# jirsat/wavenets

Measured on NVIDIA B200. Metric: audio samples/sec fwd+bwd WaveNet stack, higher is better.
Workload: dtype bf16

## Files before the change

wavenets_b200/csrc/gemm_tc_block.cuh:

```cuda
#pragma once
#include "gemm_tc.cuh"

template <int NT1> __device__ __forceinline__ void blk_tile(int pos, int n, int& kind, int& j) {
  if (pos < NT1) { kind = pos; j = 0; return; }
  const int q = (pos - NT1) / (NT1 + 1), r = (pos - NT1) % (NT1 + 1);
  if (q >= n - 1) { kind = NT1; j = n - 1; return; }
  if (r == 0) { kind = 0; j = q + 1; }
  else if (r == 1) { kind = NT1; j = q; }
  else { kind = r - 1; j = q + 1; }
}

struct TcBlockParams {
  int B, T, tiles_t, num_mtiles;
  int nseg, shift[TC_MAX_TAPS];
  int Cin, D, R, has_res;
  const float* bias_g; const float* cbias; const float* bias_r;
  unsigned long long pol_a, pol_w, pol_z, pol_g, pol_o;
  float drop_scale;
};

template <int D_, int R_> struct TcBlockCfg {
  static constexpr int BM = 128, BK = 64, BN = 256;
  static constexpr int A_BYTES = BM * BK * 2;
  static constexpr int B_BYTES = (BN / 2) * BK * 2;
  static constexpr int STAGE_BYTES = A_BYTES + B_BYTES;
  static constexpr int STAGES = 4;
  static constexpr int G_BYTES = BM * D_ * 2;
  static constexpr int PANEL = 128 * 64;
  static constexpr int OUT_SLOTS = 2, SLOT_PANELS = 2;
  static constexpr int NT1 = 2 * D_ / BN;
  static constexpr int TMEM_COLS = 512;
  static constexpr int SMEM_BYTES = STAGES * STAGE_BYTES + G_BYTES + OUT_SLOTS * SLOT_PANELS * PANEL + 512  + 2048 ;
  static_assert(D_ % 128 == 0 && D_ <= 256 && R_ % 64 == 0 && R_ <= 256, "fused block kernel: D in {128,256}, R <= 256");
  static_assert(SMEM_BYTES <= 232448, "fused block kernel does not fit shared memory");
};

template <int D_, int R_>
__global__ void __launch_bounds__(384, 1)
tc_block_fwd_kernel(const __grid_constant__ CUtensorMap tmA, const __grid_constant__ CUtensorMap tmX, const __grid_constant__ CUtensorMap tmW1,
                    const __grid_constant__ CUtensorMap tmW2, const __grid_constant__ CUtensorMap tmZf, const __grid_constant__ CUtensorMap tmZs,
                    const __grid_constant__ CUtensorMap tmG, const __grid_constant__ CUtensorMap tmO, const TcBlockParams p) {
  using Cfg = TcBlockCfg<D_, R_>;
  constexpr int STAGES = Cfg::STAGES, NEPI = 8, NT1 = Cfg::NT1;
  constexpr int KB_G = D_ / 64, KB_X = R_ / 64;
  extern __shared__ __align__(1024) uint8_t smem_blk[];
  uint8_t* smem = smem_blk;
  if ((smem_u32(smem) & 1023u) != 0u) { if (threadIdx.x == 0) printf("libwavenet_b200: dynamic shared memory is not 1024-byte aligned\n"); __trap(); }
  uint8_t* gbuf = smem + STAGES * Cfg::STAGE_BYTES;
  uint8_t* out_ring = gbuf + Cfg::G_BYTES;
  uint64_t* full_bar = (uint64_t*)(out_ring + Cfg::OUT_SLOTS * Cfg::SLOT_PANELS * Cfg::PANEL);
  uint64_t* empty_bar = full_bar + STAGES;
  uint64_t* tfull_bar = empty_bar + STAGES;
  uint64_t* tempty_bar = tfull_bar + 2;
  uint64_t* out_empty = tempty_bar + 2;
  uint64_t* g_done = out_empty + Cfg::OUT_SLOTS;
  uint64_t* g_full = g_done + 1;
  uint64_t* g_free = g_full + 1;
  uint64_t* g_cons = g_free + 1;
  uint32_t* tmem_ptr = (uint32_t*)(g_cons + 2);
  float* bias_s = (float*)(((uintptr_t)(tmem_ptr + 4) + 15) & ~(uintptr_t)15);

  const int warp = threadIdx.x >> 5, lane = threadIdx.x & 31;
  const uint32_t crank = cluster_ctarank();
  const bool leader = crank == 0;
  const int tile_first = (int)blockIdx.x >> 1, tile_stride = (int)gridDim.x >> 1;
  const int pair_row0 = (int)crank * Cfg::BM;
  const int kb_a = p.Cin / 64;
  const int n_mt = tile_first < p.num_mtiles ? (p.num_mtiles - tile_first + tile_stride - 1) / tile_stride : 0;
  const int n_pos = n_mt * (NT1 + 1);

  if (warp == 0 && lane == 0) {
    tma_prefetch_desc(&tmA); tma_prefetch_desc(&tmW1); tma_prefetch_desc(&tmW2); tma_prefetch_desc(&tmX);
  }
  if (warp == 1 && lane == 0) {
    for (int i = 0; i < STAGES; ++i) { mbar_init(&full_bar[i], 1); mbar_init(&empty_bar[i], 1); }
    for (int i = 0; i < 2; ++i) { mbar_init(&tfull_bar[i], 1); mbar_init(&tempty_bar[i], NEPI * 2); }
    for (int i = 0; i < Cfg::OUT_SLOTS; ++i) mbar_init(&out_empty[i], 1);
    mbar_init(g_done, NEPI); mbar_init(g_full, 2); mbar_init(g_free, 1); mbar_init(&g_cons[0], 1); mbar_init(&g_cons[1], 1);
    mbar_fence_init();
  }
  if (warp == 2) tmem_alloc_pair<Cfg::TMEM_COLS>(tmem_ptr);
  tc_fence_before();
  __syncthreads();
  cluster_sync_all();
  tc_fence_after();
  const uint32_t tmem_base = *tmem_ptr;
  pdl_launch_dependents();
  pdl_wait();

  if (warp == 0) {
    if (lane == 0) {
      int stage = 0; uint32_t phase = 0;
      auto next = [&]() { if (++stage == STAGES) { stage = 0; phase ^= 1; } };
      constexpr int W2_BYTES = (R_ / 2) * 64 * 2;
      for (int pos = 0; pos < n_pos; ++pos) {
// ... 2 lines not shown
        const int mt = tile_first + j * tile_stride;
        const int b = mt / p.tiles_t, t0 = (mt % p.tiles_t) * (2 * Cfg::BM) + pair_row0;
        if (kind < NT1) {
          int wk = 0;
          for (int s = 0; s < p.nseg; ++s) {
            for (int kb = 0; kb < kb_a; ++kb) {
              mbar_wait(&empty_bar[stage], phase ^ 1);
              uint8_t* sa = smem + stage * Cfg::STAGE_BYTES;
              if (leader) mbar_expect_tx(&full_bar[stage], 2 * Cfg::STAGE_BYTES);
              tma_load_4d_pair_h(sa, &tmA, &full_bar[stage], kb * 64, t0 + p.shift[s], b, 0, p.pol_a);
              tma_load_2d_pair_h(sa + Cfg::A_BYTES, &tmW1, &full_bar[stage], wk + kb * 64, kind * Cfg::BN + (int)crank * (Cfg::BN / 2), p.pol_w);
              next();
            }
            wk += p.Cin;
          }
        } else {
          for (int kb = 0; kb < KB_G; ++kb) {
            mbar_wait(&empty_bar[stage], phase ^ 1);
            uint8_t* sa = smem + stage * Cfg::STAGE_BYTES;
            if (leader) mbar_expect_tx(&full_bar[stage], 2 * W2_BYTES);
            tma_load_2d_pair_h(sa + Cfg::A_BYTES, &tmW2, &full_bar[stage], kb * 64, (int)crank * (R_ / 2), p.pol_w);
            next();
          }
          if (p.has_res) {
            for (int kb = 0; kb < KB_X; ++kb) {
              mbar_wait(&empty_bar[stage], phase ^ 1);
              uint8_t* sa = smem + stage * Cfg::STAGE_BYTES;
              if (leader) mbar_expect_tx(&full_bar[stage], 2 * (Cfg::A_BYTES + W2_BYTES));
              tma_load_4d_pair_h(sa, &tmX, &full_bar[stage], kb * 64, t0, b, 0, p.pol_a);
              tma_load_2d_pair_h(sa + Cfg::A_BYTES, &tmW2, &full_bar[stage], D_ + kb * 64, (int)crank * (R_ / 2), p.pol_w);
              next();
            }
          }
        }
      }
    }
  } else if (warp == 1) {
    if (leader) {
      constexpr uint32_t idesc_g = umma_idesc_bf16(256, Cfg::BN, 0, 0);
      constexpr uint32_t idesc_o = umma_idesc_bf16(256, R_, 0, 0);
      int stage = 0; uint32_t phase = 0;
      int as = 0; uint32_t aphase = 0;
      uint32_t gphase = 0;
      const int ksteps_g = p.nseg * kb_a;
      const int ksteps_o = KB_G + (p.has_res ? KB_X : 0);
#ifdef TC_TIMELINE
      long long tl_rec[12][4]; int tl_n = 0; const long long tl_start = clock64();
#endif
      for (int pos = 0; pos < n_pos; ++pos) {
        {
          int kind, j;
          blk_tile<NT1>(pos, n_mt, kind, j);
          const bool is_out = kind == NT1;
          const int ksteps = is_out ? ksteps_o : ksteps_g;
#ifdef TC_TIMELINE
          const long long tl0 = clock64();
#endif
          mbar_wait(&tempty_bar[as], aphase ^ 1);
#ifdef TC_TIMELINE
          const long long tl1 = clock64();
#endif
          if (is_out) { mbar_wait(g_full, gphase); gphase ^= 1; }
#ifdef TC_TIMELINE
          const long long tl2 = clock64();
#endif
          tc_fence_after();
          const uint32_t d_tmem = tmem_base + (uint32_t)(as * Cfg::BN);
          for (int ks = 0; ks < ksteps; ++ks) {
            mbar_wait(&full_bar[stage], phase);
            tc_fence_after();
            if (elect_one()) {
              const uint32_t sa = smem_u32(smem + stage * Cfg::STAGE_BYTES);
              const uint32_t a_addr = (is_out && ks < KB_G) ? smem_u32(gbuf) + (uint32_t)ks * (uint32_t)Cfg::A_BYTES : sa;
              const uint64_t adesc = umma_smem_desc(a_addr, 16, 1024);
              const uint64_t bdesc = umma_smem_desc(sa + Cfg::A_BYTES, 16, 1024);
#pragma unroll
              for (int k = 0; k < Cfg::BK / 16; ++k)
                umma_bf16_pair(d_tmem, adesc + (uint64_t)(2 * k), bdesc + (uint64_t)(2 * k), is_out ? idesc_o : idesc_g, (ks | k) != 0);
              umma_commit_pair(&empty_bar[stage]);
              if (ks == ksteps - 1) umma_commit_pair(&tfull_bar[as]);
              if (is_out && ks < KB_G && (ks + 1) % (KB_G / NT1) == 0) umma_commit_pair(&g_cons[(ks + 1) / (KB_G / NT1) - 1]);
            }
            __syncwarp();
            if (++stage == STAGES) { stage = 0; phase ^= 1; }
          }
#ifdef TC_TIMELINE
          if (tl_n < 12) { tl_rec[tl_n][0] = tl1 - tl0; tl_rec[tl_n][1] = tl2 - tl1; tl_rec[tl_n][2] = clock64() - tl2; tl_rec[tl_n][3] = tl0 - tl_start; ++tl_n; }
#endif
          if (++as == 2) { as = 0; aphase ^= 1; }
        }
      }
#ifdef TC_TIMELINE
      if (blockIdx.x == 0 && lane == 0)
        for (int i = 0; i < tl_n; ++i) printf("BLK mma tile %d: t0 %lld wait_tempty %lld wait_g %lld issue %lld\n", i, tl_rec[i][3], tl_rec[i][0], tl_rec[i][1], tl_rec[i][2]);
#endif
    }
  } else if (warp == 2) {
    int oslot = 0, prev = -1;
    auto step_store = [&](const CUtensorMap* m0, const CUtensorMap* m1, int c0, int t0, int b, unsigned long long pol) {
      named_bar_sync(3 + oslot, NEPI * 32 + 32);
      if (lane == 0) {
        const uint8_t* ob = out_ring + oslot * Cfg::SLOT_PANELS * Cfg::PANEL;
        tma_store_3d_h(ob, m0, c0, t0, b, pol);
        if (m1) tma_store_3d_h(ob + Cfg::PANEL, m1, c0, t0, b, pol);
// ... 47 lines not shown
    const uint32_t u0 = (uint32_t)(2 * q), u1 = u0 + 1;
    const uint32_t off0 = row_off + ((u0 ^ sw) << 4), off1 = row_off + ((u1 ^ sw) << 4);
    const uint32_t grow = (uint32_t)row * 128u, gsw = (uint32_t)(row & 7);
    int as = 0; uint32_t aphase = 0;
    int oslot = 0; uint32_t ophase = 0;

#ifdef TC_TIMELINE
    long long tl_rec[12][3]; int tl_n = 0; const long long tl_start = clock64();
#endif
    const TcEpiGate<true>::Params pg{p.bias_g, p.cbias, D_};
    const TcEpiBiasActRes<true>::Params po{p.bias_r, nullptr, 0, ACT_LINEAR, R_};
    for (int pos = 0; pos < n_pos; ++pos) {
      int nt, j;
      blk_tile<NT1>(pos, n_mt, nt, j);
      const int mt = tile_first + j * tile_stride;
      const int b = mt / p.tiles_t;
      const int bsafe = b < p.B ? b : p.B - 1;
      {
        const bool is_out = nt == NT1;
        const int tid = (int)threadIdx.x - 128;
        float bias_reg = 0.f;
        if (is_out) { if (tid < R_) bias_reg = TcEpiBiasActRes<true>::bias_load(po, bsafe, 0, R_, tid); }
        else bias_reg = TcEpiGate<true>::bias_load(pg, bsafe, nt * (Cfg::BN / 2), Cfg::BN, tid);
#ifdef TC_TIMELINE
        const long long te0 = clock64();
#endif
        mbar_wait(&tfull_bar[as], aphase);
        tc_fence_after();
#ifdef TC_TIMELINE
        const long long te1 = clock64();
#endif
        float* const bs = bias_s + as * 256;
        bs[tid] = bias_reg;
        named_bar_sync(2, NEPI * 32);
        TmemAccRow acc{tmem_base + (uint32_t)(as * Cfg::BN) + ((uint32_t)(quarter * 32) << 16), true};
        if (!is_out) {
          if (j > 0) {
            mbar_wait(&g_cons[nt], (uint32_t)((j - 1) & 1));
            if (nt == 0) mbar_wait(g_free, (uint32_t)((j - 1) & 1));
          }
#pragma unroll 1
          for (int step = 0; step < Cfg::BN / 64; ++step) {
            float in[1][16];
            float out[3][16];
            TcEpiGate<true>::chunk(pg, acc, bsafe, step * 32 + q * 16, Cfg::BN / 2, 0, 0u, in, out, bs);
            uint8_t* ob = out_ring + oslot * Cfg::SLOT_PANELS * Cfg::PANEL;
// ... 12 lines not shown
              const int ch = nt * (Cfg::BN / 2) + step * 32 + q * 16;
              uint8_t* gs = gbuf + (ch >> 6) * Cfg::A_BYTES + grow;
              const uint32_t j0 = (uint32_t)((ch & 63) >> 3);
              uint4 a, c;
              a.x = pack_bf16x2(out[2][0], out[2][1]); a.y = pack_bf16x2(out[2][2], out[2][3]);
              a.z = pack_bf16x2(out[2][4], out[2][5]); a.w = pack_bf16x2(out[2][6], out[2][7]);
              c.x = pack_bf16x2(out[2][8], out[2][9]); c.y = pack_bf16x2(out[2][10], out[2][11]);
              c.z = pack_bf16x2(out[2][12], out[2][13]); c.w = pack_bf16x2(out[2][14], out[2][15]);
              *reinterpret_cast<uint4*>(gs + ((j0 ^ gsw) << 4)) = a;
              *reinterpret_cast<uint4*>(gs + (((j0 + 1) ^ gsw) << 4)) = c;
            }
            fence_proxy_async();
            named_bar_arrive(3 + oslot, NEPI * 32 + 32);
            if (++oslot == Cfg::OUT_SLOTS) { oslot = 0; ophase ^= 1; }
          }
          if (nt == NT1 - 1) {
            named_bar_arrive(8, NEPI * 32 + 32);
            __syncwarp();
            if (lane == 0) mbar_arrive(g_done);
          }
        } else {
#pragma unroll 1
          for (int step = 0; step < R_ / 32; ++step) {
            float in[1][16];
            float out[1][16];
            TcEpiBiasActRes<true>::chunk(po, acc, bsafe, step * 32 + q * 16, 0, 0, 0u, in, out, bs);
            uint8_t* ob = out_ring + oslot * Cfg::SLOT_PANELS * Cfg::PANEL;
            mbar_wait(&out_empty[oslot], ophase ^ 1);
            uint4 a, c;
            a.x = pack_bf16x2(out[0][0], out[0][1]); a.y = pack_bf16x2(out[0][2], out[0][3]);
            a.z = pack_bf16x2(out[0][4], out[0][5]); a.w = pack_bf16x2(out[0][6], out[0][7]);
            c.x = pack_bf16x2(out[0][8], out[0][9]); c.y = pack_bf16x2(out[0][10], out[0][11]);
            c.z = pack_bf16x2(out[0][12], out[0][13]); c.w = pack_bf16x2(out[0][14], out[0][15]);
            *reinterpret_cast<uint4*>(ob + off0) = a;
            *reinterpret_cast<uint4*>(ob + off1) = c;
            fence_proxy_async();
            named_bar_arrive(3 + oslot, NEPI * 32 + 32);
            if (++oslot == Cfg::OUT_SLOTS) { oslot = 0; ophase ^= 1; }
          }
        }
#ifdef TC_TIMELINE
        if (tl_n < 12) { tl_rec[tl_n][0] = te1 - te0; tl_rec[tl_n][1] = clock64() - te1; tl_rec[tl_n][2] = te0 - tl_start; ++tl_n; }
#endif
        tc_fence_before();
        __syncwarp();
        if (lane == 0) mbar_arrive_remote_relaxed(&tempty_bar[as], 0u);
        if (++as == 2) { as = 0; aphase ^= 1; }
      }
    }
// ... 11 lines not shown
struct TcBlockDesc {
  int B, T, nseg, shift[TC_MAX_TAPS], Cin, D, R, has_res;
  const bf16* A; int lda;
  const bf16* X; int ldx;
  const bf16* W1; int k1;
  const bf16* W2;
  bf16* z; bf16* g; bf16* xout;
  const float* bias_g; const float* cbias; const float* bias_r;
  const uint8_t* mask_next; bf16* xdrop_next; float drop_scale;
  int plain, act;
};

static inline const CUtensorMap* tc_slab_map(TmapCache& tc, const bf16* base, int ld, int C, int T, int B) {
  uint64_t dims[3] = {(uint64_t)C, (uint64_t)T, (uint64_t)B};
  uint64_t str[2] = {(uint64_t)ld * 2, (uint64_t)T * ld * 2};
  uint32_t box[3] = {64, 128, 1};
  return tc.get(base, 3, dims, str, box, 128);
}

template <int D_, int R_>
static int tc_block_fwd_launch(TmapCache& tc, cudaStream_t st, const TcBlockDesc& d) {
  using Cfg = TcBlockCfg<D_, R_>;
  const CUtensorMap* mA = tc_act_map(tc, d.A, d.lda, d.Cin, d.T, d.B, 1, 0, 128);
  const CUtensorMap* mX = tc_act_map(tc, d.X, d.ldx, d.R, d.T, d.B, 1, 0, 128);
  uint64_t w1d[2] = {(uint64_t)d.k1, (uint64_t)(2 * d.D)}, w1s[1] = {(uint64_t)d.k1 * 2};
  uint32_t w1b[2] = {64, 128};
  const CUtensorMap* mW1 = tc.get(d.W1, 2, w1d, w1s, w1b);
  uint64_t w2d[2] = {(uint64_t)(d.D + d.R), (uint64_t)d.R}, w2s[1] = {(uint64_t)(d.D + d.R) * 2};
  uint32_t w2b[2] = {64, (uint32_t)(R_ / 2)};
  const CUtensorMap* mW2 = tc.get(d.W2, 2, w2d, w2s, w2b);
  const TcEpiIo zf{d.z, 2 * d.D, d.D, 0}, zs{d.z + d.D, 2 * d.D, d.D, 0}, xo{d.xout, d.R, d.R, 0};
  const CUtensorMap* mZf = tc_panel_map(tc, zf, d.T, d.B);
  const CUtensorMap* mZs = tc_panel_map(tc, zs, d.T, d.B);
  const CUtensorMap* mO = tc_panel_map(tc, xo, d.T, d.B);
  const CUtensorMap* mG = tc_slab_map(tc, d.g, d.D, d.D, d.T, d.B);
  if (!mA || !mX || !mW1 || !mW2 || !mZf || !mZs || !mO || !mG) return -10;
  TcBlockParams p{};
  p.B = d.B; p.T = d.T; p.tiles_t = (d.T + 255) / 256; p.num_mtiles = d.B * p.tiles_t;
  p.nseg = d.nseg;
  for (int s = 0; s < d.nseg; ++s) p.shift[s] = d.shift[s];
  p.Cin = d.Cin; p.D = d.D; p.R = d.R; p.has_res = d.has_res;
  p.bias_g = d.bias_g; p.cbias = d.cbias; p.bias_r = d.bias_r;
  p.pol_a = tc_policy(TC_L2_NORMAL); p.pol_w = tc_policy(TC_L2_LAST);
  p.pol_z = tc_policy(TC_L2_FIRST); p.pol_g = tc_policy(TC_L2_FIRST); p.pol_o = tc_policy(TC_L2_LAST);
  auto kern = tc_block_fwd_kernel<D_, R_>;
  static unsigned long long attr_devs = 0ull;
  if (tc_first_use_on_device(&attr_devs)) {
    cudaError_t e = cudaFuncSetAttribute(kern, cudaFuncAttributeMaxDynamicSharedMemorySize, Cfg::SMEM_BYTES);
    if (e != cudaSuccess) { snprintf(g_tc_err, sizeof(g_tc_err), "cudaFuncSetAttribute(smem=%d): %s", Cfg::SMEM_BYTES, cudaGetErrorString(e)); return -12; }
  }
  const int slots = tc_balanced_slots(p.num_mtiles, tc_num_sms() / 2);
  const int grid = (p.num_mtiles < slots ? p.num_mtiles : slots) * 2;
  cudaLaunchConfig_t cfg{};
  cfg.gridDim = dim3(grid); cfg.blockDim = dim3(384); cfg.dynamicSmemBytes = Cfg::SMEM_BYTES; cfg.stream = st;
  cudaLaunchAttribute attr[2];
  cfg.attrs = attr; cfg.numAttrs = tc_launch_attrs(attr, 2);
  cudaError_t e = cudaLaunchKernelEx(&cfg, kern, *mA, *mX, *mW1, *mW2, *mZf, *mZs, *mG, *mO, p);
  if (e != cudaSuccess) { snprintf(g_tc_err, sizeof(g_tc_err), "fused block forward launch: %s", cudaGetErrorString(e)); return -13; }
  return 0;
}

static inline int tc_block_fwd(TmapCache& tc, cudaStream_t st, const TcBlockDesc& d) {
  if (d.Cin % 64 != 0 || d.nseg < 1 || d.nseg > TC_MAX_TAPS) return -100;
  if (d.D == 256 && d.R == 256) return tc_block_fwd_launch<256, 256>(tc, st, d);
  if (d.D == 128 && d.R == 128) return tc_block_fwd_launch<128, 128>(tc, st, d);
  return -100;
}
```

wavenets_b200/csrc/gemm_tc_stack.cuh:

```cuda
#pragma once
#include "gemm_tc_block.cuh"

#ifdef TC_TIMELINE
#define SFT_DECL(n) long long sft[n] = {}; long long sft_prev = clock64();
#define SFT(i) { const long long sft_now = clock64(); sft[i] += sft_now - sft_prev; sft_prev = sft_now; }
#else
#define SFT_DECL(n)
#define SFT(i)
#endif

#define TC_STACK_MAX_LAYERS 256
struct alignas(128) TcStackLayer {
  CUtensorMap tmA, tmX, tmW1, tmW2, tmZf, tmZs, tmG, tmO, tmOd;
  int shift[TC_MAX_TAPS];
  const float* bias_g; const float* cbias; const float* bias_r;
  const uint8_t* mask_next;
  int kind;
  int act;
};

template <int NT1> struct TcStackSeq {
  const uint32_t* kmask; int n, tile_first, tile_stride, num_mtiles;
  int j, ph, r;
  __device__ __forceinline__ TcStackSeq(const uint32_t* km, int n_, int tf, int ts, int nm) : kmask(km), n(n_), tile_first(tf), tile_stride(ts), num_mtiles(nm), j(0), ph(0), r(1) {}
  __device__ __forceinline__ bool plain(int jj) const {
    const int ly = (tile_first + jj * tile_stride) / num_mtiles;
    return ((kmask[ly >> 5] >> (ly & 31)) & 1u) != 0u;
  }
  __device__ __forceinline__ bool next(int& kind, int& jj) {
    for (;;) {
      switch (ph) {
        case 0:
          if (n <= 0) return false;
          ph = 1; r = 1; kind = plain(0) ? NT1 + 1 : 0; jj = 0; return true;
        case 1:
          if (!plain(0) && r < NT1) { kind = r++; jj = 0; return true; }
          ph = 2; j = 0; break;
        case 2:
// ... 1 lines not shown
          if (j + 1 < n) { kind = plain(j + 1) ? NT1 + 1 : 0; jj = j + 1; return true; }
          break;
        case 3:
          ph = 4; r = 1;
          if (!plain(j)) { kind = NT1; jj = j; return true; }
          break;
        default:
          if (j + 1 < n && !plain(j + 1) && r < NT1) { kind = r++; jj = j + 1; return true; }
          if (++j >= n) return false;
          ph = 2; break;
      }
    }
  }
};

__device__ __forceinline__ int ld_acquire_gpu(const int* p) {
  int v;
  asm volatile("ld.acquire.gpu.global.s32 %0, [%1];" : "=r"(v) : "l"(p) : "memory");
  return v;
}
__device__ __forceinline__ void red_release_gpu_add(int* p, int v) {
  asm volatile("red.release.gpu.global.add.s32 [%0], %1;" ::"l"(p), "r"(v) : "memory");
}
__device__ __forceinline__ void fence_proxy_async_global() { asm volatile("fence.proxy.async.global;" ::: "memory"); }

template <int D_, int R_>
__global__ void __launch_bounds__(384, 1)
tc_stack_fwd_kernel(const TcStackLayer* __restrict__ layers, const int L, int* __restrict__ flags, const TcBlockParams p) {

  using Cfg = TcBlockCfg<D_, R_>;
  constexpr int STAGES = Cfg::STAGES, NEPI = 8, NT1 = Cfg::NT1;
  constexpr int KB_G = D_ / 64, KB_X = R_ / 64;
  extern __shared__ __align__(1024) uint8_t smem_blk[];
  uint8_t* smem = smem_blk;
  if ((smem_u32(smem) & 1023u) != 0u) { if (threadIdx.x == 0) printf("libwavenet_b200: dynamic shared memory is not 1024-byte aligned\n"); __trap(); }
  uint8_t* gbuf = smem + STAGES * Cfg::STAGE_BYTES;
  uint8_t* out_ring = gbuf + Cfg::G_BYTES;
  uint64_t* full_bar = (uint64_t*)(out_ring + Cfg::OUT_SLOTS * Cfg::SLOT_PANELS * Cfg::PANEL);
  uint64_t* empty_bar = full_bar + STAGES;
  uint64_t* tfull_bar = empty_bar + STAGES;
  uint64_t* tempty_bar = tfull_bar + 2;
  uint64_t* out_empty = tempty_bar + 2;
  uint64_t* g_done = out_empty + Cfg::OUT_SLOTS;
  uint64_t* g_full = g_done + 1;
  uint64_t* g_free = g_full + 1;
  uint64_t* g_cons = g_free + 1;
  uint32_t* tmem_ptr = (uint32_t*)(g_cons + 2);
  float* bias_s = (float*)(((uintptr_t)(tmem_ptr + 4) + 15) & ~(uintptr_t)15);
  uint32_t* kmask = (uint32_t*)(bias_s + 512);

  const int warp = threadIdx.x >> 5, lane = threadIdx.x & 31;
  const uint32_t crank = cluster_ctarank();
  const bool leader = crank == 0;
  const int tile_first = (int)blockIdx.x >> 1, tile_stride = (int)gridDim.x >> 1;
  const int pair_row0 = (int)crank * Cfg::BM;
  const int kb_a = p.Cin / 64;
  const int total_tiles = L * p.num_mtiles;
  const int n_mt = tile_first < total_tiles ? (total_tiles - tile_first + tile_stride - 1) / tile_stride : 0;
  constexpr int K_OUT = NT1, K_PLAIN = NT1 + 1;

  if (warp == 0 && lane == 0 && n_mt > 0) {
    const TcStackLayer& L0 = layers[tile_first / p.num_mtiles];
    tma_prefetch_desc(&L0.tmA); tma_prefetch_desc(&L0.tmW1); tma_prefetch_desc(&L0.tmW2); tma_prefetch_desc(&L0.tmX);
  }
  if (warp == 1 && lane == 0) {
    for (int i = 0; i < STAGES; ++i) { mbar_init(&full_bar[i], 1); mbar_init(&empty_bar[i], 1); }
    for (int i = 0; i < 2; ++i) { mbar_init(&tfull_bar[i], 1); mbar_init(&tempty_bar[i], NEPI * 2); }
    for (int i = 0; i < Cfg::OUT_SLOTS; ++i) mbar_init(&out_empty[i], 1);
    mbar_init(g_done, NEPI); mbar_init(g_full, 2); mbar_init(g_free, 1); mbar_init(&g_cons[0], 1); mbar_init(&g_cons[1], 1);
    mbar_fence_init();
  }
  if (warp == 2) tmem_alloc_pair<Cfg::TMEM_COLS>(tmem_ptr);
  if (threadIdx.x >= 128 && threadIdx.x < 128 + TC_STACK_MAX_LAYERS / 32) {
    const int w = (int)threadIdx.x - 128;
    uint32_t m = 0u;
    for (int l = w * 32; l < L && l < w * 32 + 32; ++l) if (layers[l].kind != 0) m |= 1u << (l & 31);
    kmask[w] = m;
  }
  tc_fence_before();
  __syncthreads();
  cluster_sync_all();
  tc_fence_after();
  const uint32_t tmem_base = *tmem_ptr;
  pdl_launch_dependents();
  pdl_wait();

  if (warp == 0) {
    if (lane == 0) {
      int stage = 0; uint32_t phase = 0;
      auto next = [&]() { if (++stage == STAGES) { stage = 0; phase ^= 1; } };
      constexpr int W2_BYTES = (R_ / 2) * 64 * 2;
      TcStackSeq<NT1> seq(kmask, n_mt, tile_first, tile_stride, p.num_mtiles);
      int kind, j;
// ... 5 lines not shown
        SFT(0)
        if (kind != K_OUT) {
          const int wrow = kind == K_PLAIN ? 0 : kind * Cfg::BN;
          if ((kind == 0 || kind == K_PLAIN) && ly > 0) {
            const int tb = mt % p.tiles_t, row0 = tb * (2 * Cfg::BM);
            const int* fl = flags + (size_t)(ly - 1) * p.num_mtiles + (mt - tb);
            for (int s = 0; s < p.nseg; ++s) {
              const int lo = row0 + Ly.shift[s], hi = lo + 2 * Cfg::BM - 1;
              if (hi < 0) continue;
              const int t_lo = lo < 0 ? 0 : lo / (2 * Cfg::BM);
              int t_hi = hi / (2 * Cfg::BM);
              if (t_hi > p.tiles_t - 1) t_hi = p.tiles_t - 1;
              for (int tt = t_lo; tt <= t_hi; ++tt) {
                const long long spin0 = clock64();
                while (ld_acquire_gpu(fl + tt) < 2) {
                  __nanosleep(32);
                  if (clock64() - spin0 > 6000000000ll) { printf("libwavenet_b200: stack forward waited > 3 s for tile (%d, %d)\n", ly - 1, mt - tb + tt); __trap(); }
                }
              }
            }
            fence_proxy_async_global();
            SFT(1)
          }
          int wk = 0;
          for (int s = 0; s < p.nseg; ++s) {
            for (int kb = 0; kb < kb_a; ++kb) {
              mbar_wait(&empty_bar[stage], phase ^ 1);
              uint8_t* sa = smem + stage * Cfg::STAGE_BYTES;
              if (leader) mbar_expect_tx(&full_bar[stage], 2 * Cfg::STAGE_BYTES);
              tma_load_4d_pair_h(sa, &Ly.tmA, &full_bar[stage], kb * 64, t0 + Ly.shift[s], b, 0, p.pol_a);
              tma_load_2d_pair_h(sa + Cfg::A_BYTES, &Ly.tmW1, &full_bar[stage], wk + kb * 64, wrow + (int)crank * (Cfg::BN / 2), p.pol_w);
              next();
            }
            wk += p.Cin;
          }
        } else {
          for (int kb = 0; kb < KB_G; ++kb) {
            mbar_wait(&empty_bar[stage], phase ^ 1);
            uint8_t* sa = smem + stage * Cfg::STAGE_BYTES;
            if (leader) mbar_expect_tx(&full_bar[stage], 2 * W2_BYTES);
            tma_load_2d_pair_h(sa + Cfg::A_BYTES, &Ly.tmW2, &full_bar[stage], kb * 64, (int)crank * (R_ / 2), p.pol_w);
            next();
          }
          if (p.has_res) {
            for (int kb = 0; kb < KB_X; ++kb) {
              mbar_wait(&empty_bar[stage], phase ^ 1);
              uint8_t* sa = smem + stage * Cfg::STAGE_BYTES;
              if (leader) mbar_expect_tx(&full_bar[stage], 2 * (Cfg::A_BYTES + W2_BYTES));
              tma_load_4d_pair_h(sa, &Ly.tmX, &full_bar[stage], kb * 64, t0, b, 0, p.pol_a);
              tma_load_2d_pair_h(sa + Cfg::A_BYTES, &Ly.tmW2, &full_bar[stage], D_ + kb * 64, (int)crank * (R_ / 2), p.pol_w);
              next();
            }
          }
        }
      }
      SFT(0)
#ifdef TC_TIMELINE
      if (blockIdx.x == 0 || blockIdx.x == 41) printf("SFWD cta %d producer: tiles %d  ring+issue %lld  wait_flags %lld\n", blockIdx.x, n_mt, sft[0], sft[1]);
#endif
    }
  } else if (warp == 1) {
    if (leader) {
      constexpr uint32_t idesc_g = umma_idesc_bf16(256, Cfg::BN, 0, 0);
      constexpr uint32_t idesc_o = umma_idesc_bf16(256, R_, 0, 0);
      int stage = 0; uint32_t phase = 0;
      int as = 0; uint32_t aphase = 0;
      uint32_t gphase = 0;
      const int ksteps_g = p.nseg * kb_a;
      const int ksteps_o = KB_G + (p.has_res ? KB_X : 0);
      TcStackSeq<NT1> seq(kmask, n_mt, tile_first, tile_stride, p.num_mtiles);
      int kind, j;
      SFT_DECL(8)
      while (seq.next(kind, j)) {
        {
          const bool is_out = kind == K_OUT;
          const int ksteps = is_out ? ksteps_o : ksteps_g;
          SFT(0)
          mbar_wait(&tempty_bar[as], aphase ^ 1);
          SFT(1)
          if (is_out) { mbar_wait(g_full, gphase); gphase ^= 1; }
          SFT(2)
          tc_fence_after();
          const uint32_t d_tmem = tmem_base + (uint32_t)(as * Cfg::BN);
          for (int ks = 0; ks < ksteps; ++ks) {
            mbar_wait(&full_bar[stage], phase);
            SFT(3)
            tc_fence_after();
            if (elect_one()) {
              const uint32_t sa = smem_u32(smem + stage * Cfg::STAGE_BYTES);
              const uint32_t a_addr = (is_out && ks < KB_G) ? smem_u32(gbuf) + (uint32_t)ks * (uint32_t)Cfg::A_BYTES : sa;
              const uint64_t adesc = umma_smem_desc(a_addr, 16, 1024);
              const uint64_t bdesc = umma_smem_desc(sa + Cfg::A_BYTES, 16, 1024);
#pragma unroll
              for (int k = 0; k < Cfg::BK / 16; ++k)
                umma_bf16_pair(d_tmem, adesc + (uint64_t)(2 * k), bdesc + (uint64_t)(2 * k), is_out ? idesc_o : idesc_g, (ks | k) != 0);
              umma_commit_pair(&empty_bar[stage]);
              if (ks == ksteps - 1) umma_commit_pair(&tfull_bar[as]);
              if (is_out && ks < KB_G && (ks + 1) % (KB_G / NT1) == 0) umma_commit_pair(&g_cons[(ks + 1) / (KB_G / NT1) - 1]);
            }
            __syncwarp();
            if (++stage == STAGES) { stage = 0; phase ^= 1; }
          }
          if (++as == 2) { as = 0; aphase ^= 1; }
        }
      }
#ifdef TC_TIMELINE
      if (lane == 0 && (blockIdx.x == 0 || blockIdx.x == 40))
        printf("SFWD cta %d mma: tiles %d  wait_tempty %lld  wait_g_full %lld  wait_full_bar %lld  issue+other %lld\n", blockIdx.x, n_mt, sft[1], sft[2], sft[3], sft[0]);
#endif
    }
  } else if (warp == 2) {
    int oslot = 0, prev = -1, pend_flag = -1, pend_new = -1;
    const bool delay_publish = p.num_mtiles > 2 * tile_stride;
    auto step_store = [&](const CUtensorMap* m0, const CUtensorMap* m1, int c0, int t0, int b, unsigned long long pol) {
      named_bar_sync(3 + oslot, NEPI * 32 + 32);
      if (lane == 0) {
        const uint8_t* ob = out_ring + oslot * Cfg::SLOT_PANELS * Cfg::PANEL;
        tma_store_3d_h(ob, m0, c0, t0, b, pol);
        if (m1) tma_store_3d_h(ob + Cfg::PANEL, m1, c0, t0, b, pol);
        bulk_commit_group();
        if (prev >= 0) { bulk_wait_group_read<1>(); mbar_arrive(&out_empty[prev]); }
// ... 84 lines not shown
    int ng = 0, ng_j = -1;
    SFT_DECL(8)

    TcStackSeq<NT1> seq(kmask, n_mt, tile_first, tile_stride, p.num_mtiles);
    int nt, j;
    while (seq.next(nt, j)) {
      const int gt = tile_first + j * tile_stride, ly = gt / p.num_mtiles, mt = gt - ly * p.num_mtiles;
      const TcStackLayer& Ly = layers[ly];
      const int b = mt / p.tiles_t;
      const int bsafe = b < p.B ? b : p.B - 1;
      const bool is_plain = nt == K_PLAIN;
      if (nt == 0) {
        if (ng_j >= 0) ++ng;
        ng_j = j;
      }
      const TcEpiGate<true>::Params pg{Ly.bias_g, Ly.cbias, D_};
      const TcEpiBiasActRes<true>::Params po{is_plain ? Ly.bias_g : Ly.bias_r, nullptr, 0, is_plain ? Ly.act : ACT_LINEAR, is_plain ? Cfg::BN : R_};
      {
        const bool is_out = nt == K_OUT || is_plain;
        const int tid = (int)threadIdx.x - 128;
        float bias_reg = 0.f;
        if (is_out) { if (tid < po.N) bias_reg = TcEpiBiasActRes<true>::bias_load(po, bsafe, 0, po.N, tid); }
        else bias_reg = TcEpiGate<true>::bias_load(pg, bsafe, nt * (Cfg::BN / 2), Cfg::BN, tid);
#ifdef TC_TIMELINE
        const int wb = is_plain ? 7 : (nt == K_OUT ? 6 : 5);
#endif
        SFT(4)
        mbar_wait(&tfull_bar[as], aphase);
        SFT(1)
        tc_fence_after();
        float* const bs = bias_s + as * 256;
        bs[tid] = bias_reg;
        named_bar_sync(2, NEPI * 32);
        TmemAccRow acc{tmem_base + (uint32_t)(as * Cfg::BN) + ((uint32_t)(quarter * 32) << 16), true};
        if (!is_out) {
          if (ng > 0) {
            SFT(wb)
            mbar_wait(&g_cons[nt], (uint32_t)((ng - 1) & 1));
            if (nt == 0) mbar_wait(g_free, (uint32_t)((ng - 1) & 1));
            SFT(2)
          }
#pragma unroll 1
          for (int step = 0; step < Cfg::BN / 64; ++step) {
            float in[1][16];
            float out[3][16];
            TcEpiGate<true>::chunk(pg, acc, bsafe, step * 32 + q * 16, Cfg::BN / 2, 0, 0u, in, out, bs);
// ... 16 lines not shown
              uint8_t* gs = gbuf + (ch >> 6) * Cfg::A_BYTES + grow;
              const uint32_t j0 = (uint32_t)((ch & 63) >> 3);
              uint4 a, c;
              a.x = pack_bf16x2(out[2][0], out[2][1]); a.y = pack_bf16x2(out[2][2], out[2][3]);
              a.z = pack_bf16x2(out[2][4], out[2][5]); a.w = pack_bf16x2(out[2][6], out[2][7]);
              c.x = pack_bf16x2(out[2][8], out[2][9]); c.y = pack_bf16x2(out[2][10], out[2][11]);
              c.z = pack_bf16x2(out[2][12], out[2][13]); c.w = pack_bf16x2(out[2][14], out[2][15]);
              *reinterpret_cast<uint4*>(gs + ((j0 ^ gsw) << 4)) = a;
              *reinterpret_cast<uint4*>(gs + (((j0 + 1) ^ gsw) << 4)) = c;
            }
            fence_proxy_async();
            named_bar_arrive(3 + oslot, NEPI * 32 + 32);
            if (++oslot == Cfg::OUT_SLOTS) { oslot = 0; ophase ^= 1; }
          }
          if (nt == NT1 - 1) {
            named_bar_arrive(8, NEPI * 32 + 32);
            __syncwarp();
            if (lane == 0) mbar_arrive(g_done);
          }
        } else {
          const uint8_t* const mask_next = is_plain ? nullptr : Ly.mask_next;
#pragma unroll 1
          for (int step = 0; step < po.N / 32; ++step) {
            float in[1][16];
            float out[1][16];
            TcEpiBiasActRes<true>::chunk(po, acc, bsafe, step * 32 + q * 16, 0, 0, 0u, in, out, bs);
            uint4 mk = make_uint4(0u, 0u, 0u, 0u);
            if (mask_next) {
              const int tt = (mt % p.tiles_t) * (2 * Cfg::BM) + pair_row0 + row;
              if (tt < p.T && b < p.B)
                mk = __ldg(reinterpret_cast<const uint4*>(mask_next + ((size_t)b * p.T + tt) * R_ + step * 32 + q * 16));
            }
            uint8_t* ob = out_ring + oslot * Cfg::SLOT_PANELS * Cfg::PANEL;
            SFT(wb)
            mbar_wait(&out_empty[oslot], ophase ^ 1);
            SFT(3)
            uint4 a, c;
            a.x = pack_bf16x2(out[0][0], out[0][1]); a.y = pack_bf16x2(out[0][2], out[0][3]);
            a.z = pack_bf16x2(out[0][4], out[0][5]); a.w = pack_bf16x2(out[0][6], out[0][7]);
            c.x = pack_bf16x2(out[0][8], out[0][9]); c.y = pack_bf16x2(out[0][10], out[0][11]);
            c.z = pack_bf16x2(out[0][12], out[0][13]); c.w = pack_bf16x2(out[0][14], out[0][15]);
            *reinterpret_cast<uint4*>(ob + off0) = a;
            *reinterpret_cast<uint4*>(ob + off1) = c;
            if (mask_next) {
              const uint32_t xw[8] = {a.x, a.y, a.z, a.w, c.x, c.y, c.z, c.w};
              const uint32_t mw[4] = {mk.x, mk.y, mk.z, mk.w};
              uint32_t dw[8];
#pragma unroll
              for (int i = 0; i < 8; ++i) {
// ... 33 lines not shown


struct TcStackPlan {
  int B = 0, T = 0, L = 0, num_mtiles = 0; bool cb = false, drop = false;
  TcStackLayer* d_layers = nullptr; int* d_flags = nullptr;
  void release() { cudaFree(d_layers); cudaFree(d_flags); d_layers = nullptr; d_flags = nullptr; }
};

template <int D_, int R_>
static int tc_stack_build_t(TmapCache& tc, const std::vector<TcBlockDesc>& descs, TcStackPlan* plan) {
  std::vector<TcStackLayer> tab(descs.size());
  for (size_t l = 0; l < descs.size(); ++l) {
    const TcBlockDesc& d = descs[l];
    TcStackLayer& t = tab[l];
    memset(&t, 0, sizeof(t));
    const CUtensorMap* mA = tc_act_map(tc, d.A, d.lda, d.Cin, d.T, d.B, 1, 0, 128);
    uint64_t w1d[2] = {(uint64_t)d.k1, (uint64_t)(d.plain ? d.D : 2 * d.D)}, w1s[1] = {(uint64_t)d.k1 * 2};
    uint32_t w1b[2] = {64, 128};
    const CUtensorMap* mW1 = tc.get(d.W1, 2, w1d, w1s, w1b);
    const TcEpiIo xo{d.xout, d.plain ? d.D : d.R, d.plain ? d.D : d.R, 0};
    const CUtensorMap* mO = tc_panel_map(tc, xo, d.T, d.B);
    if (!mA || !mW1 || !mO) return -10;
    t.tmA = *mA; t.tmW1 = *mW1; t.tmO = *mO; t.tmOd = *mO;
    t.tmX = *mA; t.tmW2 = *mW1; t.tmZf = *mO; t.tmZs = *mO; t.tmG = *mO;
    t.kind = d.plain ? 1 : 0; t.act = d.act;
    if (!d.plain) {
      const CUtensorMap* mX = tc_act_map(tc, d.X, d.ldx, d.R, d.T, d.B, 1, 0, 128);
      uint64_t w2d[2] = {(uint64_t)(d.D + d.R), (uint64_t)d.R}, w2s[1] = {(uint64_t)(d.D + d.R) * 2};
      uint32_t w2b[2] = {64, (uint32_t)(R_ / 2)};
      const CUtensorMap* mW2 = tc.get(d.W2, 2, w2d, w2s, w2b);
      const TcEpiIo zf{d.z, 2 * d.D, d.D, 0}, zs{d.z + d.D, 2 * d.D, d.D, 0};
      const CUtensorMap* mZf = tc_panel_map(tc, zf, d.T, d.B);
      const CUtensorMap* mZs = tc_panel_map(tc, zs, d.T, d.B);
      const CUtensorMap* mG = tc_slab_map(tc, d.g, d.D, d.D, d.T, d.B);
      if (!mX || !mW2 || !mZf || !mZs || !mG) return -10;
      t.tmX = *mX; t.tmW2 = *mW2; t.tmZf = *mZf; t.tmZs = *mZs; t.tmG = *mG;
      if (d.mask_next && d.xdrop_next) {
        const TcEpiIo xd{d.xdrop_next, d.R, d.R, 0};
        const CUtensorMap* mOd = tc_panel_map(tc, xd, d.T, d.B);
        if (!mOd) return -10;
        t.tmOd = *mOd; t.mask_next = d.mask_next;
      }
    }
    for (int s = 0; s < TC_MAX_TAPS; ++s) t.shift[s] = s < d.nseg ? d.shift[s] : 0;
    t.bias_g = d.bias_g; t.cbias = d.cbias; t.bias_r = d.bias_r;
  }
  const TcBlockDesc& d0 = descs[0];
  if (descs.size() > TC_STACK_MAX_LAYERS) return -100;
  plan->release();
  plan->B = d0.B; plan->T = d0.T; plan->L = (int)descs.size(); plan->num_mtiles = d0.B * ((d0.T + 255) / 256); plan->cb = false; plan->drop = false;
  for (const TcBlockDesc& d : descs) { if (d.cbias) plan->cb = true; if (d.mask_next) plan->drop = true; }
  if (cudaMalloc((void**)&plan->d_layers, tab.size() * sizeof(TcStackLayer)) != cudaSuccess ||
      cudaMemcpy(plan->d_layers, tab.data(), tab.size() * sizeof(TcStackLayer), cudaMemcpyHostToDevice) != cudaSuccess ||
      cudaMalloc((void**)&plan->d_flags, (size_t)plan->L * plan->num_mtiles * sizeof(int)) != cudaSuccess) {
    snprintf(g_tc_err, sizeof(g_tc_err), "stack forward: plan allocation failed: %s", cudaGetErrorString(cudaGetLastError()));
    plan->release();
    return -23;
  }
  return 0;
// ... 60 lines not shown
```

Baseline: 11.22 million.

## Add residual input in epilogue instead of identity-matrix GEMM k-steps

The residual connection was previously computed by extra MMA k-steps that multiplied the residual input X by an identity-like block in W2, requiring TMA loads of X and extra W2 columns. The epilogue warps now load X rows directly from global memory with a small register prefetch ring and add them to the accumulator alongside the bias. This removes KB_X pipeline stages of TMA traffic and tensor-core work per output tile. In the persistent stack kernel it adds a shared-memory acquire/release flag so epilogue threads wait until the producer has confirmed the previous layer's X is ready, which adds a spin-wait and extra register pressure.

```diff
diff --git a/wavenets_b200/csrc/gemm_tc_block.cuh b/wavenets_b200/csrc/gemm_tc_block.cuh
--- a/wavenets_b200/csrc/gemm_tc_block.cuh
+++ b/wavenets_b200/csrc/gemm_tc_block.cuh
@@ -15,6 +15,7 @@
   int nseg, shift[TC_MAX_TAPS];
   int Cin, D, R, has_res;
   const float* bias_g; const float* cbias; const float* bias_r;
+  const bf16* x; int ldx;
   unsigned long long pol_a, pol_w, pol_z, pol_g, pol_o;
   float drop_scale;
 };
@@ -35,14 +36,31 @@
   static_assert(SMEM_BYTES <= 232448, "fused block kernel does not fit shared memory");
 };
 
+template <class Acc>
+__device__ __forceinline__ void blk_out16(Acc& acc, int c, bool has_x, const uint4 (&x)[2], const float* bs, float* v) {
+  acc.load16(c, v);
+  if (has_x) {
+    const uint32_t xw[8] = {x[0].x, x[0].y, x[0].z, x[0].w, x[1].x, x[1].y, x[1].z, x[1].w};
+#pragma unroll
+    for (int i = 0; i < 8; ++i) {
+      v[2 * i] += __uint_as_float(xw[i] << 16);
+      v[2 * i + 1] += __uint_as_float(xw[i] & 0xffff0000u);
+    }
+  }
+  float t[16];
+  ld_bias16(bs + c, t);
+#pragma unroll
+  for (int i = 0; i < 16; ++i) v[i] += t[i];
+}
+
 template <int D_, int R_>
 __global__ void __launch_bounds__(384, 1)
-tc_block_fwd_kernel(const __grid_constant__ CUtensorMap tmA, const __grid_constant__ CUtensorMap tmX, const __grid_constant__ CUtensorMap tmW1,
+tc_block_fwd_kernel(const __grid_constant__ CUtensorMap tmA, const __grid_constant__ CUtensorMap tmW1,
                     const __grid_constant__ CUtensorMap tmW2, const __grid_constant__ CUtensorMap tmZf, const __grid_constant__ CUtensorMap tmZs,
                     const __grid_constant__ CUtensorMap tmG, const __grid_constant__ CUtensorMap tmO, const TcBlockParams p) {
   using Cfg = TcBlockCfg<D_, R_>;
   constexpr int STAGES = Cfg::STAGES, NEPI = 8, NT1 = Cfg::NT1;
-  constexpr int KB_G = D_ / 64, KB_X = R_ / 64;
+  constexpr int KB_G = D_ / 64;
   extern __shared__ __align__(1024) uint8_t smem_blk[];
   uint8_t* smem = smem_blk;
   if ((smem_u32(smem) & 1023u) != 0u) { if (threadIdx.x == 0) printf("libwavenet_b200: dynamic shared memory is not 1024-byte aligned\n"); __trap(); }
@@ -70,7 +88,7 @@
   const int n_pos = n_mt * (NT1 + 1);
 
   if (warp == 0 && lane == 0) {
-    tma_prefetch_desc(&tmA); tma_prefetch_desc(&tmW1); tma_prefetch_desc(&tmW2); tma_prefetch_desc(&tmX);
+    tma_prefetch_desc(&tmA); tma_prefetch_desc(&tmW1); tma_prefetch_desc(&tmW2);
   }
   if (warp == 1 && lane == 0) {
     for (int i = 0; i < STAGES; ++i) { mbar_init(&full_bar[i], 1); mbar_init(&empty_bar[i], 1); }
@@ -119,16 +137,6 @@
             tma_load_2d_pair_h(sa + Cfg::A_BYTES, &tmW2, &full_bar[stage], kb * 64, (int)crank * (R_ / 2), p.pol_w);
             next();
           }
-          if (p.has_res) {
-            for (int kb = 0; kb < KB_X; ++kb) {
-              mbar_wait(&empty_bar[stage], phase ^ 1);
-              uint8_t* sa = smem + stage * Cfg::STAGE_BYTES;
-              if (leader) mbar_expect_tx(&full_bar[stage], 2 * (Cfg::A_BYTES + W2_BYTES));
-              tma_load_4d_pair_h(sa, &tmX, &full_bar[stage], kb * 64, t0, b, 0, p.pol_a);
-              tma_load_2d_pair_h(sa + Cfg::A_BYTES, &tmW2, &full_bar[stage], D_ + kb * 64, (int)crank * (R_ / 2), p.pol_w);
-              next();
-            }
-          }
         }
       }
     }
@@ -140,7 +148,6 @@
       int as = 0; uint32_t aphase = 0;
       uint32_t gphase = 0;
       const int ksteps_g = p.nseg * kb_a;
-      const int ksteps_o = KB_G + (p.has_res ? KB_X : 0);
 #ifdef TC_TIMELINE
       long long tl_rec[12][4]; int tl_n = 0; const long long tl_start = clock64();
 #endif
@@ -149,7 +156,7 @@
           int kind, j;
           blk_tile<NT1>(pos, n_mt, kind, j);
           const bool is_out = kind == NT1;
-          const int ksteps = is_out ? ksteps_o : ksteps_g;
+          const int ksteps = is_out ? KB_G : ksteps_g;
 #ifdef TC_TIMELINE
           const long long tl0 = clock64();
 #endif
@@ -168,7 +175,7 @@
             tc_fence_after();
             if (elect_one()) {
               const uint32_t sa = smem_u32(smem + stage * Cfg::STAGE_BYTES);
-              const uint32_t a_addr = (is_out && ks < KB_G) ? smem_u32(gbuf) + (uint32_t)ks * (uint32_t)Cfg::A_BYTES : sa;
+              const uint32_t a_addr = is_out ? smem_u32(gbuf) + (uint32_t)ks * (uint32_t)Cfg::A_BYTES : sa;
               const uint64_t adesc = umma_smem_desc(a_addr, 16, 1024);
               const uint64_t bdesc = umma_smem_desc(sa + Cfg::A_BYTES, 16, 1024);
 #pragma unroll
@@ -176,7 +183,7 @@
                 umma_bf16_pair(d_tmem, adesc + (uint64_t)(2 * k), bdesc + (uint64_t)(2 * k), is_out ? idesc_o : idesc_g, (ks | k) != 0);
               umma_commit_pair(&empty_bar[stage]);
               if (ks == ksteps - 1) umma_commit_pair(&tfull_bar[as]);
-              if (is_out && ks < KB_G && (ks + 1) % (KB_G / NT1) == 0) umma_commit_pair(&g_cons[(ks + 1) / (KB_G / NT1) - 1]);
+              if (is_out && (ks + 1) % (KB_G / NT1) == 0) umma_commit_pair(&g_cons[(ks + 1) / (KB_G / NT1) - 1]);
             }
             __syncwarp();
             if (++stage == STAGES) { stage = 0; phase ^= 1; }
@@ -270,6 +277,22 @@
         float bias_reg = 0.f;
         if (is_out) { if (tid < R_) bias_reg = TcEpiBiasActRes<true>::bias_load(po, bsafe, 0, R_, tid); }
         else bias_reg = TcEpiGate<true>::bias_load(pg, bsafe, nt * (Cfg::BN / 2), Cfg::BN, tid);
+        bool has_x = false;
+        constexpr int XQ = R_ / 32 < 4 ? R_ / 32 : 4;
+        const bf16* xrow = nullptr;
+        uint4 xq[XQ][2];
+        if (is_out && p.has_res) {
+          const int tt = (mt % p.tiles_t) * (2 * Cfg::BM) + pair_row0 + row;
+          if (tt < p.T) {
+            xrow = p.x + ((size_t)b * p.T + tt) * p.ldx + q * 16;
+#pragma unroll
+            for (int st = 0; st < XQ; ++st) {
+              xq[st][0] = __ldg(reinterpret_cast<const uint4*>(xrow + st * 32));
+              xq[st][1] = __ldg(reinterpret_cast<const uint4*>(xrow + st * 32 + 8));
+            }
+            has_x = true;
+          }
+        }
 #ifdef TC_TIMELINE
         const long long te0 = clock64();
 #endif
@@ -328,9 +351,15 @@
         } else {
 #pragma unroll 1
           for (int step = 0; step < R_ / 32; ++step) {
-            float in[1][16];
+            const uint4 xc[2] = {xq[0][0], xq[0][1]};
+#pragma unroll
+            for (int st = 0; st + 1 < XQ; ++st) { xq[st][0] = xq[st + 1][0]; xq[st][1] = xq[st + 1][1]; }
+            if (has_x && step + XQ < R_ / 32) {
+              xq[XQ - 1][0] = __ldg(reinterpret_cast<const uint4*>(xrow + (step + XQ) * 32));
+              xq[XQ - 1][1] = __ldg(reinterpret_cast<const uint4*>(xrow + (step + XQ) * 32 + 8));
+            }
             float out[1][16];
-            TcEpiBiasActRes<true>::chunk(po, acc, bsafe, step * 32 + q * 16, 0, 0, 0u, in, out, bs);
+            blk_out16(acc, step * 32 + q * 16, has_x, xc, bs, out[0]);
             uint8_t* ob = out_ring + oslot * Cfg::SLOT_PANELS * Cfg::PANEL;
             mbar_wait(&out_empty[oslot], ophase ^ 1);
             uint4 a, c;
@@ -388,11 +417,10 @@
 static int tc_block_fwd_launch(TmapCache& tc, cudaStream_t st, const TcBlockDesc& d) {
   using Cfg = TcBlockCfg<D_, R_>;
   const CUtensorMap* mA = tc_act_map(tc, d.A, d.lda, d.Cin, d.T, d.B, 1, 0, 128);
-  const CUtensorMap* mX = tc_act_map(tc, d.X, d.ldx, d.R, d.T, d.B, 1, 0, 128);
   uint64_t w1d[2] = {(uint64_t)d.k1, (uint64_t)(2 * d.D)}, w1s[1] = {(uint64_t)d.k1 * 2};
   uint32_t w1b[2] = {64, 128};
   const CUtensorMap* mW1 = tc.get(d.W1, 2, w1d, w1s, w1b);
-  uint64_t w2d[2] = {(uint64_t)(d.D + d.R), (uint64_t)d.R}, w2s[1] = {(uint64_t)(d.D + d.R) * 2};
+  uint64_t w2d[2] = {(uint64_t)d.D, (uint64_t)d.R}, w2s[1] = {(uint64_t)(d.D + d.R) * 2};
   uint32_t w2b[2] = {64, (uint32_t)(R_ / 2)};
   const CUtensorMap* mW2 = tc.get(d.W2, 2, w2d, w2s, w2b);
   const TcEpiIo zf{d.z, 2 * d.D, d.D, 0}, zs{d.z + d.D, 2 * d.D, d.D, 0}, xo{d.xout, d.R, d.R, 0};
@@ -400,13 +428,14 @@
   const CUtensorMap* mZs = tc_panel_map(tc, zs, d.T, d.B);
   const CUtensorMap* mO = tc_panel_map(tc, xo, d.T, d.B);
   const CUtensorMap* mG = tc_slab_map(tc, d.g, d.D, d.D, d.T, d.B);
-  if (!mA || !mX || !mW1 || !mW2 || !mZf || !mZs || !mO || !mG) return -10;
+  if (!mA || !mW1 || !mW2 || !mZf || !mZs || !mO || !mG) return -10;
   TcBlockParams p{};
   p.B = d.B; p.T = d.T; p.tiles_t = (d.T + 255) / 256; p.num_mtiles = d.B * p.tiles_t;
   p.nseg = d.nseg;
   for (int s = 0; s < d.nseg; ++s) p.shift[s] = d.shift[s];
   p.Cin = d.Cin; p.D = d.D; p.R = d.R; p.has_res = d.has_res;
   p.bias_g = d.bias_g; p.cbias = d.cbias; p.bias_r = d.bias_r;
+  p.x = d.X; p.ldx = d.ldx;
   p.pol_a = tc_policy(TC_L2_NORMAL); p.pol_w = tc_policy(TC_L2_LAST);
   p.pol_z = tc_policy(TC_L2_FIRST); p.pol_g = tc_policy(TC_L2_FIRST); p.pol_o = tc_policy(TC_L2_LAST);
   auto kern = tc_block_fwd_kernel<D_, R_>;
@@ -421,7 +450,7 @@
   cfg.gridDim = dim3(grid); cfg.blockDim = dim3(384); cfg.dynamicSmemBytes = Cfg::SMEM_BYTES; cfg.stream = st;
   cudaLaunchAttribute attr[2];
   cfg.attrs = attr; cfg.numAttrs = tc_launch_attrs(attr, 2);
-  cudaError_t e = cudaLaunchKernelEx(&cfg, kern, *mA, *mX, *mW1, *mW2, *mZf, *mZs, *mG, *mO, p);
+  cudaError_t e = cudaLaunchKernelEx(&cfg, kern, *mA, *mW1, *mW2, *mZf, *mZs, *mG, *mO, p);
   if (e != cudaSuccess) { snprintf(g_tc_err, sizeof(g_tc_err), "fused block forward launch: %s", cudaGetErrorString(e)); return -13; }
   return 0;
 }
diff --git a/wavenets_b200/csrc/gemm_tc_stack.cuh b/wavenets_b200/csrc/gemm_tc_stack.cuh
--- a/wavenets_b200/csrc/gemm_tc_stack.cuh
+++ b/wavenets_b200/csrc/gemm_tc_stack.cuh
@@ -11,9 +11,11 @@
 
 #define TC_STACK_MAX_LAYERS 256
 struct alignas(128) TcStackLayer {
-  CUtensorMap tmA, tmX, tmW1, tmW2, tmZf, tmZs, tmG, tmO, tmOd;
+  CUtensorMap tmA, tmW1, tmW2, tmZf, tmZs, tmG, tmO, tmOd;
   int shift[TC_MAX_TAPS];
   const float* bias_g; const float* cbias; const float* bias_r;
+  const bf16* x; int ldx;
+  int x_layer;
   const uint8_t* mask_next;
   int kind;
   int act;
@@ -61,6 +63,14 @@
 __device__ __forceinline__ void red_release_gpu_add(int* p, int v) {
   asm volatile("red.release.gpu.global.add.s32 [%0], %1;" ::"l"(p), "r"(v) : "memory");
 }
+__device__ __forceinline__ void st_release_cta_shared(uint32_t* p, uint32_t v) {
+  asm volatile("st.release.cta.shared::cta.u32 [%0], %1;" ::"r"(smem_u32(p)), "r"(v) : "memory");
+}
+__device__ __forceinline__ uint32_t ld_acquire_cta_shared(const uint32_t* p) {
+  uint32_t v;
+  asm volatile("ld.acquire.cta.shared::cta.u32 %0, [%1];" : "=r"(v) : "r"(smem_u32(p)) : "memory");
+  return v;
+}
 __device__ __forceinline__ void fence_proxy_async_global() { asm volatile("fence.proxy.async.global;" ::: "memory"); }
 
 template <int D_, int R_>
@@ -69,7 +79,7 @@
 
   using Cfg = TcBlockCfg<D_, R_>;
   constexpr int STAGES = Cfg::STAGES, NEPI = 8, NT1 = Cfg::NT1;
-  constexpr int KB_G = D_ / 64, KB_X = R_ / 64;
+  constexpr int KB_G = D_ / 64;
   extern __shared__ __align__(1024) uint8_t smem_blk[];
   uint8_t* smem = smem_blk;
   if ((smem_u32(smem) & 1023u) != 0u) { if (threadIdx.x == 0) printf("libwavenet_b200: dynamic shared memory is not 1024-byte aligned\n"); __trap(); }
@@ -87,6 +97,7 @@
   uint32_t* tmem_ptr = (uint32_t*)(g_cons + 2);
   float* bias_s = (float*)(((uintptr_t)(tmem_ptr + 4) + 15) & ~(uintptr_t)15);
   uint32_t* kmask = (uint32_t*)(bias_s + 512);
+  uint32_t* x_ready = kmask + TC_STACK_MAX_LAYERS / 32;
 
   const int warp = threadIdx.x >> 5, lane = threadIdx.x & 31;
   const uint32_t crank = cluster_ctarank();
@@ -100,7 +111,7 @@
 
   if (warp == 0 && lane == 0 && n_mt > 0) {
     const TcStackLayer& L0 = layers[tile_first / p.num_mtiles];
-    tma_prefetch_desc(&L0.tmA); tma_prefetch_desc(&L0.tmW1); tma_prefetch_desc(&L0.tmW2); tma_prefetch_desc(&L0.tmX);
+    tma_prefetch_desc(&L0.tmA); tma_prefetch_desc(&L0.tmW1); tma_prefetch_desc(&L0.tmW2);
   }
   if (warp == 1 && lane == 0) {
     for (int i = 0; i < STAGES; ++i) { mbar_init(&full_bar[i], 1); mbar_init(&empty_bar[i], 1); }
@@ -108,6 +119,7 @@
     for (int i = 0; i < Cfg::OUT_SLOTS; ++i) mbar_init(&out_empty[i], 1);
     mbar_init(g_done, NEPI); mbar_init(g_full, 2); mbar_init(g_free, 1); mbar_init(&g_cons[0], 1); mbar_init(&g_cons[1], 1);
     mbar_fence_init();
+    *x_ready = 0u;
   }
   if (warp == 2) tmem_alloc_pair<Cfg::TMEM_COLS>(tmem_ptr);
   if (threadIdx.x >= 128 && threadIdx.x < 128 + TC_STACK_MAX_LAYERS / 32) {
@@ -159,6 +171,7 @@
             fence_proxy_async_global();
             SFT(1)
           }
+          if (kind == 0 || kind == K_PLAIN) st_release_cta_shared(x_ready, (uint32_t)j + 1u);
           int wk = 0;
           for (int s = 0; s < p.nseg; ++s) {
             for (int kb = 0; kb < kb_a; ++kb) {
@@ -179,16 +192,6 @@
             tma_load_2d_pair_h(sa + Cfg::A_BYTES, &Ly.tmW2, &full_bar[stage], kb * 64, (int)crank * (R_ / 2), p.pol_w);
             next();
           }
-          if (p.has_res) {
-            for (int kb = 0; kb < KB_X; ++kb) {
-              mbar_wait(&empty_bar[stage], phase ^ 1);
-              uint8_t* sa = smem + stage * Cfg::STAGE_BYTES;
-              if (leader) mbar_expect_tx(&full_bar[stage], 2 * (Cfg::A_BYTES + W2_BYTES));
-              tma_load_4d_pair_h(sa, &Ly.tmX, &full_bar[stage], kb * 64, t0, b, 0, p.pol_a);
-              tma_load_2d_pair_h(sa + Cfg::A_BYTES, &Ly.tmW2, &full_bar[stage], D_ + kb * 64, (int)crank * (R_ / 2), p.pol_w);
-              next();
-            }
-          }
         }
       }
       SFT(0)
@@ -204,14 +207,13 @@
       int as = 0; uint32_t aphase = 0;
       uint32_t gphase = 0;
       const int ksteps_g = p.nseg * kb_a;
-      const int ksteps_o = KB_G + (p.has_res ? KB_X : 0);
       TcStackSeq<NT1> seq(kmask, n_mt, tile_first, tile_stride, p.num_mtiles);
       int kind, j;
       SFT_DECL(8)
       while (seq.next(kind, j)) {
         {
           const bool is_out = kind == K_OUT;
-          const int ksteps = is_out ? ksteps_o : ksteps_g;
+          const int ksteps = is_out ? KB_G : ksteps_g;
           SFT(0)
           mbar_wait(&tempty_bar[as], aphase ^ 1);
           SFT(1)
@@ -225,7 +227,7 @@
             tc_fence_after();
             if (elect_one()) {
               const uint32_t sa = smem_u32(smem + stage * Cfg::STAGE_BYTES);
-              const uint32_t a_addr = (is_out && ks < KB_G) ? smem_u32(gbuf) + (uint32_t)ks * (uint32_t)Cfg::A_BYTES : sa;
+              const uint32_t a_addr = is_out ? smem_u32(gbuf) + (uint32_t)ks * (uint32_t)Cfg::A_BYTES : sa;
               const uint64_t adesc = umma_smem_desc(a_addr, 16, 1024);
               const uint64_t bdesc = umma_smem_desc(sa + Cfg::A_BYTES, 16, 1024);
 #pragma unroll
@@ -233,7 +235,7 @@
                 umma_bf16_pair(d_tmem, adesc + (uint64_t)(2 * k), bdesc + (uint64_t)(2 * k), is_out ? idesc_o : idesc_g, (ks | k) != 0);
               umma_commit_pair(&empty_bar[stage]);
               if (ks == ksteps - 1) umma_commit_pair(&tfull_bar[as]);
-              if (is_out && ks < KB_G && (ks + 1) % (KB_G / NT1) == 0) umma_commit_pair(&g_cons[(ks + 1) / (KB_G / NT1) - 1]);
+              if (is_out && (ks + 1) % (KB_G / NT1) == 0) umma_commit_pair(&g_cons[(ks + 1) / (KB_G / NT1) - 1]);
             }
             __syncwarp();
             if (++stage == STAGES) { stage = 0; phase ^= 1; }
@@ -364,6 +366,23 @@
         float bias_reg = 0.f;
         if (is_out) { if (tid < po.N) bias_reg = TcEpiBiasActRes<true>::bias_load(po, bsafe, 0, po.N, tid); }
         else bias_reg = TcEpiGate<true>::bias_load(pg, bsafe, nt * (Cfg::BN / 2), Cfg::BN, tid);
+        bool has_x = false;
+        constexpr int XQ = R_ / 32 < 4 ? R_ / 32 : 4;
+        const bf16* xrow = nullptr;
+        uint4 xq[XQ][2];
+        if (nt == K_OUT && p.has_res) {
+          const int tt = (mt % p.tiles_t) * (2 * Cfg::BM) + pair_row0 + row;
+          if (tt < p.T && b < p.B) {
+            if (Ly.x_layer >= 0) while (ld_acquire_cta_shared(x_ready) < (uint32_t)j + 1u) {}
+            xrow = Ly.x + ((size_t)b * p.T + tt) * Ly.ldx + q * 16;
+#pragma unroll
+            for (int st = 0; st < XQ; ++st) {
+              xq[st][0] = __ldcg(reinterpret_cast<const uint4*>(xrow + st * 32));
+              xq[st][1] = __ldcg(reinterpret_cast<const uint4*>(xrow + st * 32 + 8));
+            }
+            has_x = true;
+          }
+        }
 #ifdef TC_TIMELINE
         const int wb = is_plain ? 7 : (nt == K_OUT ? 6 : 5);
 #endif
@@ -426,9 +445,17 @@
           const uint8_t* const mask_next = is_plain ? nullptr : Ly.mask_next;
 #pragma unroll 1
           for (int step = 0; step < po.N / 32; ++step) {
+            const uint4 xc[2] = {xq[0][0], xq[0][1]};
+#pragma unroll
+            for (int st = 0; st + 1 < XQ; ++st) { xq[st][0] = xq[st + 1][0]; xq[st][1] = xq[st + 1][1]; }
+            if (has_x && step + XQ < R_ / 32) {
+              xq[XQ - 1][0] = __ldcg(reinterpret_cast<const uint4*>(xrow + (step + XQ) * 32));
+              xq[XQ - 1][1] = __ldcg(reinterpret_cast<const uint4*>(xrow + (step + XQ) * 32 + 8));
+            }
             float in[1][16];
             float out[1][16];
-            TcEpiBiasActRes<true>::chunk(po, acc, bsafe, step * 32 + q * 16, 0, 0, 0u, in, out, bs);
+            if (is_plain) TcEpiBiasActRes<true>::chunk(po, acc, bsafe, step * 32 + q * 16, 0, 0, 0u, in, out, bs);
+            else blk_out16(acc, step * 32 + q * 16, has_x, xc, bs, out[0]);
             uint4 mk = make_uint4(0u, 0u, 0u, 0u);
             if (mask_next) {
               const int tt = (mt % p.tiles_t) * (2 * Cfg::BM) + pair_row0 + row;
@@ -508,19 +535,20 @@
     const CUtensorMap* mO = tc_panel_map(tc, xo, d.T, d.B);
     if (!mA || !mW1 || !mO) return -10;
     t.tmA = *mA; t.tmW1 = *mW1; t.tmO = *mO; t.tmOd = *mO;
-    t.tmX = *mA; t.tmW2 = *mW1; t.tmZf = *mO; t.tmZs = *mO; t.tmG = *mO;
+    t.tmW2 = *mW1; t.tmZf = *mO; t.tmZs = *mO; t.tmG = *mO;
     t.kind = d.plain ? 1 : 0; t.act = d.act;
     if (!d.plain) {
-      const CUtensorMap* mX = tc_act_map(tc, d.X, d.ldx, d.R, d.T, d.B, 1, 0, 128);
-      uint64_t w2d[2] = {(uint64_t)(d.D + d.R), (uint64_t)d.R}, w2s[1] = {(uint64_t)(d.D + d.R) * 2};
+      uint64_t w2d[2] = {(uint64_t)d.D, (uint64_t)d.R}, w2s[1] = {(uint64_t)(d.D + d.R) * 2};
       uint32_t w2b[2] = {64, (uint32_t)(R_ / 2)};
       const CUtensorMap* mW2 = tc.get(d.W2, 2, w2d, w2s, w2b);
       const TcEpiIo zf{d.z, 2 * d.D, d.D, 0}, zs{d.z + d.D, 2 * d.D, d.D, 0};
       const CUtensorMap* mZf = tc_panel_map(tc, zf, d.T, d.B);
       const CUtensorMap* mZs = tc_panel_map(tc, zs, d.T, d.B);
       const CUtensorMap* mG = tc_slab_map(tc, d.g, d.D, d.D, d.T, d.B);
-      if (!mX || !mW2 || !mZf || !mZs || !mG) return -10;
-      t.tmX = *mX; t.tmW2 = *mW2; t.tmZf = *mZf; t.tmZs = *mZs; t.tmG = *mG;
+      if (!mW2 || !mZf || !mZs || !mG) return -10;
+      t.tmW2 = *mW2; t.tmZf = *mZf; t.tmZs = *mZs; t.tmG = *mG;
+      t.x = d.X; t.ldx = d.ldx; t.x_layer = -1;
+      for (size_t k = 0; k < l; ++k) if (!descs[k].plain && (const bf16*)descs[k].xout == d.X) t.x_layer = (int)k;
       if (d.mask_next && d.xdrop_next) {
         const TcEpiIo xd{d.xdrop_next, d.R, d.R, 0};
         const CUtensorMap* mOd = tc_panel_map(tc, xd, d.T, d.B);
```

Measured after the change: 10.59 million, median of 6. 5.6% lower.
